# yuanming-hu/exposure

Measured on AMD Instinct MI355X. Metric: Mpixels/s through 8-step filter chain fwd+bwd, higher is better.
Workload: dtype f16; 1 GPU; 8-step filter chain (E,G,W,S+,T,Ct,BW,C) fwd+bwd, 64x512x512x3 f16 NHWC per GPU, one HIP kernel per filter step and direction; batch_per_gpu=64, global_batch=64, height=512, width=512, parallelism=image-sharded replicas x1 (no data-path collective), weak scaling, launch=hipGraph replay, 10 steps (330 captured launches) per replay, chain_streams=2, transport=none (one process)

## Files before the change

### exposure_amd/csrc/chain_steps.hip

```cpp
#include <hip/hip_runtime.h>
#include <stdint.h>

#include "../../include/exposure_hip.h"
#include "filter_math.h"
#include "pixel_io.h"
#include "kernel_common.h"
#include "host_common.h"

namespace expo {

struct ChainStepsFwdArgs {
  const void* x;
  void* y[kChainFuseMax];
  const float* prm[kChainFuseMax];
  int id[kChainFuseMax];
  int steps, hw;
};

template <typename T, class IO>
__global__ __launch_bounds__(kThreads) void chain_steps_fwd_kernel(const ChainStepsFwdArgs a) {
  constexpr int PPL = PixTraits<T>::PPL;
  const int n = blockIdx.y;
  const int hw = a.hw;
  const size_t off = size_t(n) * hw * 3;
  const int lane = threadIdx.x & 63;
  __shared__ float2_lut ftab[kWaves][32];
  float2_lut* const tab = ftab[threadIdx.x >> 6];
#if EXPO_FP16_OVFL
  if constexpr (sizeof(T) == 2) __builtin_amdgcn_s_setreg(1 | (23 << 6) | (0 << 11), 1);
#endif
  const __amdgpu_buffer_rsrc_t rx = make_image_rsrc(static_cast<const T*>(a.x) + off, hw);
  const int stride = gridDim.x * kThreads;
  for (int gw = blockIdx.x * kThreads + (threadIdx.x & ~63); gw * PPL < hw; gw += stride) {
    const int boff = chunk_byte_offset<T>(gw, lane);
    RawGroup cur = load_raw<IO::kLoadX>(rx, boff);
#pragma unroll 1
    for (int st = 0; st < a.steps; ++st) {
      const float* const prm = a.prm[st];
      float v[PPL * 3];
#define EXPO_CASE(ID, F)                               \
  case ID: {                                           \
    const typename F::Prm q = F::load(prm + n * F::NP); \
    unpack<T>(cur, v);                                 \
    _Pragma("unroll") for (int k = 0; k < PPL; ++k) {  \
      float y[3];                                      \
      F::fwd(q, v + 3 * k, y);                         \
      _Pragma("unroll") for (int c = 0; c < 3; ++c) v[3 * k + c] = y[c]; \
    }                                                  \
    cur = pack<T>(v);                                  \
  } break;
      switch (a.id[st]) {
        EXPO_CASE(0, ExposureF)
        EXPO_CASE(1, GammaF)
        EXPO_CASE(2, WhiteBalanceF)
        EXPO_CASE(3, SatPlusF)
        case 4:
          curve_lut_build<1>(prm[n * ToneF::NP + lane % ToneF::NP], tab);
          unpack<T>(cur, v);
          curve_lut_apply<1, PPL>(v, tab);
          cur = pack<T>(v);
          __builtin_amdgcn_wave_barrier();
          break;
        EXPO_CASE(5, ContrastF)
        EXPO_CASE(6, WnbF)
        case 7:
          curve_lut_build<3>(prm[n * ColorF::NP + lane % ColorF::NP], tab);
          unpack<T>(cur, v);
          curve_lut_apply<3, PPL>(v, tab);
          cur = pack<T>(v);
          __builtin_amdgcn_wave_barrier();
          break;
        EXPO_CASE(8, LevelF)
        default: break;
      }
#undef EXPO_CASE
      store_raw<IO::kStore>(make_image_rsrc(static_cast<T*>(a.y[st]) + off, hw), boff, cur);
    }
  }
}

template <typename T>
static int chain_steps_fwd_t(const ChainStepsFwdArgs& a, int np, int h, int w, int n_geom, hipStream_t s) {
  const Geom g = make_geom<T>(n_geom, h, w, {}, kGeomMap);
  const dim3 grid(g.blocks_x, np), block(kThreads);
  if (g.stream)
    hipLaunchKernelGGL((chain_steps_fwd_kernel<T, IoStream>), grid, block, 0, s, a);
  else
    hipLaunchKernelGGL((chain_steps_fwd_kernel<T, IoCached>), grid, block, 0, s, a);
  HIP_TRY(hipGetLastError(), "chain_steps_fwd launch");
  return EXPO_OK;
}

bool chain_steps_vec_path(void* const* acts, int steps, int h, int w, int dtype) {
  const int ppv = dtype == EXPO_F16 ? VecTraits<half_t>::PPV : VecTraits<float>::PPV;
  if ((long(h) * w) % ppv != 0) return false;
  for (int k = 0; k <= steps; ++k)
    if ((reinterpret_cast<uintptr_t>(acts[k]) & 3) != 0) return false;
  return true;
}

int chain_steps_fwd(const int* ids, int cnt, void* const* acts, const float* const* params, int nb, int np, int h,
                    int w, int dtype, int n_geom, hipStream_t s) {
  if (cnt < 1 || cnt > kChainFuseMax) return fail(EXPO_E_BADARG, "chain_steps_fwd: step count");
  const size_t ioff = size_t(nb) * h * w * 3 * (dtype == EXPO_F16 ? 2 : 4);
  ChainStepsFwdArgs a{};
  a.x = static_cast<const char*>(acts[0]) + ioff;
  for (int k = 0; k < cnt; ++k) {
    a.y[k] = static_cast<char*>(acts[k + 1]) + ioff;
    a.prm[k] = params[k] + size_t(nb) * kNumParams[ids[k]];
    a.id[k] = ids[k];
  }
  a.steps = cnt;
  a.hw = h * w;
  return dtype == EXPO_F16 ? chain_steps_fwd_t<half_t>(a, np, h, w, n_geom, s)
                           : chain_steps_fwd_t<float>(a, np, h, w, n_geom, s);
}

}
```

### exposure_amd/csrc/chain_steps_bwd.hip

```cpp
#include <hip/hip_runtime.h>
#include <stdint.h>

#include "../../include/exposure_hip.h"
#include "filter_math.h"
#include "pixel_io.h"
#include "kernel_common.h"
#include "host_common.h"
#include "stream_bodies.h"
#include "chain_steps_bwd_body.h"

namespace expo {

bool chain_steps_bwd_fusable(int id, int dtype, int mode) {
  if (id == 3 && dtype == EXPO_F32 && mode == 1) return false;
  return chain_steps_bwd_acc_floats(id) > 0;
}

int chain_steps_bwd_acc_floats(int id) {
  switch (id) {
#define EXPO_CASE(ID, F) \
  case ID: return kAccParts * F::NACC;
    EXPO_RUN_FILTERS(EXPO_CASE)
#undef EXPO_CASE
  }
  return 0;
}

template <typename T, int MODE, class IO, int NS>
__global__ __launch_bounds__(kThreads EXPO_BWD_MIN_WAVES) void chain_steps_bwd_kernel(const ChainStepsBwdArgs<NS> a) {
  constexpr int PPL = PixTraits<T>::PPL;
  static_assert(PPL >= kAccParts, "kParts == kAccParts in both storage types");
  const int n = blockIdx.y;
  const int hw = a.hw;
  const size_t off = size_t(n) * hw * 3;
  const int lane = threadIdx.x & 63;
#if EXPO_FP16_OVFL
  if constexpr (sizeof(T) == 2) __builtin_amdgcn_s_setreg(1 | (23 << 6) | (0 << 11), 1);
#endif
  const int stride = gridDim.x * kThreads;
  int gw = blockIdx.x * kThreads + (threadIdx.x & ~63);
  const bool work = gw * PPL < hw;
  const __amdgpu_buffer_rsrc_t rdy = make_image_rsrc(static_cast<const T*>(a.dy) + off, hw);
  int boff = chunk_byte_offset<T>(gw, lane);
  RawGroup cur, x[NS];
  if (work) {
    cur = load_raw<IO::kLoadDy>(rdy, boff);
#pragma unroll
    for (int k = 0; k < NS; ++k)
      x[k] = load_raw<IO::kLoadX>(make_image_rsrc(static_cast<const T*>(a.x[k]) + off, hw), boff);
  }
  extern __shared__ float accs[];
  float* const mine = accs + threadIdx.x;
  for (int f = 0; f < a.acc_floats; ++f) mine[f * kThreads] = 0.f;
  if (work) {
    while (true) {
      const int gn = gw + stride;
      const bool more = gn * PPL < hw;
      const int bnext = chunk_byte_offset<T>(gn, lane);
      RawGroup nxt = cur;
      if (more) nxt = load_raw<IO::kLoadDy>(rdy, bnext);
#pragma unroll 1
      for (int st = 0; st < NS; ++st) {
        const float* const prm = a.prm[st];
        float* const lds = mine + a.acc_at[st] * kThreads;
#define EXPO_CASE(ID, F) \
  case ID: run_step<F, T, MODE>(prm + n * F::NP, x[0], cur, lds); break;
        switch (a.id[st]) {
          EXPO_RUN_FILTERS(EXPO_CASE)
          default: break;
        }
#undef EXPO_CASE
        store_raw<IO::kStore>(make_image_rsrc(static_cast<T*>(a.dx[st]) + off, hw), boff, cur);
#pragma unroll
        for (int k = 0; k + 1 < NS; ++k) x[k] = x[k + 1];
        if (more) x[NS - 1] = load_raw<IO::kLoadX>(make_image_rsrc(static_cast<const T*>(a.x[st]) + off, hw), bnext);
      }
      if (!more) break;
      gw = gn;
      boff = bnext;
      cur = nxt;
    }
  }
#pragma unroll 1
  for (int st = 0; st < NS; ++st) {
    if (st > 0) __syncthreads();
    float* const rec = a.rec[st] + size_t(n) * gridDim.x * kWsSlots;
    const float* const lds = mine + a.acc_at[st] * kThreads;
#define EXPO_CASE(ID, F) \
  case ID: run_reduce<F, T>(lds, rec); break;
    switch (a.id[st]) {
      EXPO_RUN_FILTERS(EXPO_CASE)
      default: break;
    }
#undef EXPO_CASE
  }
}

template <typename T, int MODE, int NS>
static int chain_steps_bwd_launch(const ChainStepsBwdArgs<NS>& a, const Geom& g, int np, hipStream_t s) {
  const dim3 grid(g.blocks_x, np), block(kThreads);
  const size_t lds = size_t(a.acc_floats) * kThreads * sizeof(float);
  if (g.stream)
    hipLaunchKernelGGL((chain_steps_bwd_kernel<T, MODE, IoStream, NS>), grid, block, lds, s, a);
  else
    hipLaunchKernelGGL((chain_steps_bwd_kernel<T, MODE, IoCached, NS>), grid, block, lds, s, a);
  HIP_TRY(hipGetLastError(), "chain_steps_bwd launch");
  return EXPO_OK;
}

template <typename T, int NS>
static int chain_steps_bwd_t(const int* ids, int i0, void* const* acts, void* const* grads,
                             const float* const* params, float* records, size_t step_floats, int nb, int np, int h,
                             int w, int mode, int n_geom, hipStream_t s) {
  const Geom g = make_geom<T>(n_geom, h, w, {}, kGeomReduce);
  const size_t ioff = size_t(nb) * h * w * 3 * sizeof(T);
  ChainStepsBwdArgs<NS> a{};
  a.dy = static_cast<const char*>(grads[i0 + 1]) + ioff;
  for (int k = 0; k < NS; ++k) {
    const int i = i0 - k;
    a.x[k] = static_cast<const char*>(acts[i]) + ioff;
    a.dx[k] = static_cast<char*>(grads[i]) + ioff;
    a.prm[k] = params[i] + size_t(nb) * kNumParams[ids[i]];
    a.rec[k] = records + size_t(i) * step_floats + size_t(nb) * g.blocks_x * kWsSlots;
    a.id[k] = ids[i];
    a.acc_at[k] = a.acc_floats;
    a.acc_floats += chain_steps_bwd_acc_floats(ids[i]);
  }
  a.hw = h * w;
  return mode == 1 ? chain_steps_bwd_launch<T, 1, NS>(a, g, np, s) : chain_steps_bwd_launch<T, 0, NS>(a, g, np, s);
}

int chain_steps_bwd(const int* ids, int i0, int cnt, void* const* acts, void* const* grads,
                    const float* const* params, float* records, size_t step_floats, int nb, int np, int h, int w,
                    int dtype, int mode, int n_geom, hipStream_t s) {
  if (cnt < 2 || cnt > kChainFuseMax || cnt > i0 + 1) return fail(EXPO_E_BADARG, "chain_steps_bwd: step count");
  int acc_floats = 0;
  for (int k = 0; k < cnt; ++k) {
    if (!chain_steps_bwd_fusable(ids[i0 - k], dtype, mode) || !grads[i0 - k])
      return fail(EXPO_E_BADARG, "chain_steps_bwd: not a step of the run table with a dx");
    acc_floats += chain_steps_bwd_acc_floats(ids[i0 - k]);
  }
  if (acc_floats > kChainBwdAccFloatsMax) return fail(EXPO_E_BADARG, "chain_steps_bwd: accumulators of the run");
#define EXPO_GO(NS)                                                                                                   \
  case NS:                                                                                                            \
    return dtype == EXPO_F16                                                                                          \
               ? chain_steps_bwd_t<half_t, NS>(ids, i0, acts, grads, params, records, step_floats, nb, np, h, w, mode, \
                                               n_geom, s)                                                             \
               : chain_steps_bwd_t<float, NS>(ids, i0, acts, grads, params, records, step_floats, nb, np, h, w, mode,  \
                                              n_geom, s);
  switch (cnt) {
    EXPO_GO(2) EXPO_GO(3) EXPO_GO(4) EXPO_GO(5) EXPO_GO(6) EXPO_GO(7) EXPO_GO(8)
  }
#undef EXPO_GO
  static_assert(kChainFuseMax == 8, "one instantiation per run length");
  return fail(EXPO_E_BADARG, "chain_steps_bwd: step count");
}

}
```

### exposure_amd/csrc/chain_steps_bwd_body.h

```cpp
#pragma once
#include <hip/hip_runtime.h>
#include <stdint.h>

#include "filter_math.h"
#include "pixel_io.h"
#include "kernel_common.h"
#include "stream_bodies.h"

namespace expo {

template <int NS>
struct ChainStepsBwdArgs {
  const void* dy;
  const void* x[NS];
  void* dx[NS];
  const float* prm[NS];
  float* rec[NS];
  int id[NS];
  int acc_at[NS];
  int acc_floats, hw;
};

template <class F, typename T, int MODE>
__device__ __forceinline__ void run_step(const float* prm, const RawGroup& x, RawGroup& g, float* lds) {
  constexpr int PPL = PixTraits<T>::PPL;
  constexpr int kParts = kAccParts < PPL ? kAccParts : PPL;
  static_assert(!F::kHasGroupBwd && F::kLutFloats == 0, "element-wise filters only");
  const typename F::Prm q = F::load(prm);
  float a[kParts][F::NACC];
#pragma unroll
  for (int p = 0; p < kParts; ++p)
#pragma unroll
    for (int j = 0; j < F::NACC; ++j) a[p][j] = lds[(p * F::NACC + j) * kThreads];
  float v[PPL * 3], d[PPL * 3];
  unpack<T>(x, v);
  unpack<T>(g, d);
#pragma unroll
  for (int k = 0; k < PPL; ++k) {
    float dx[3];
    F::bwd(q, nullptr, v + 3 * k, d + 3 * k, dx, a[k % kParts], MODE);
#pragma unroll
    for (int c = 0; c < 3; ++c) d[3 * k + c] = dx[c];
  }
  g = pack<T>(d);
#pragma unroll
  for (int p = 0; p < kParts; ++p)
#pragma unroll
    for (int j = 0; j < F::NACC; ++j) lds[(p * F::NACC + j) * kThreads] = a[p][j];
}

template <class F, typename T>
__device__ __forceinline__ void run_reduce(const float* lds, float* rec) {
  constexpr int PPL = PixTraits<T>::PPL;
  constexpr int kParts = kAccParts < PPL ? kAccParts : PPL;
  float acc[F::NACC];
#pragma unroll
  for (int j = 0; j < F::NACC; ++j) acc[j] = lds[j * kThreads];
#pragma unroll
  for (int p = 0; p < kParts - 1; ++p)
#pragma unroll
    for (int j = 0; j < F::NACC; ++j) acc[j] += lds[((p + 1) * F::NACC + j) * kThreads];
  block_reduce_record<F::NACC>(acc, rec);
}

#define EXPO_RUN_FILTERS(X) X(0, ExposureF) X(1, GammaF) X(2, WhiteBalanceF) X(3, SatPlusF) X(8, LevelF)

}
```

### exposure_amd/csrc/chain_steps_bwd_rc.hip

```cpp
#include <hip/hip_runtime.h>
#include <stdint.h>

#include "../../include/exposure_hip.h"
#include "filter_math.h"
#include "pixel_io.h"
#include "kernel_common.h"
#include "host_common.h"
#include "stream_bodies.h"
#include "chain_steps_bwd_body.h"

namespace expo {

#define EXPO_RC_FILTERS(X) \
  X(0, ExposureF, 1, 1) X(1, GammaF, 1, 1) X(2, WhiteBalanceF, 1, 1) X(3, SatPlusF, 1, 1) X(8, LevelF, 1, 1)

template <typename T>
__host__ __device__ constexpr bool rc_recomputable(int id) {
  switch (id) {
#define EXPO_CASE(ID, F, H, S) \
  case ID: return sizeof(T) == 2 ? H : S;
    EXPO_RC_FILTERS(EXPO_CASE)
#undef EXPO_CASE
  }
  return false;
}

template <typename T>
__host__ __device__ constexpr bool rc_keeps_load(int id) {
  switch (id) {
#define EXPO_CASE(ID, F, H, S) \
  case ID: return !(sizeof(T) == 2 ? H : S);
    EXPO_RC_FILTERS(EXPO_CASE)
#undef EXPO_CASE
  }
  return false;
}

bool chain_steps_bwd_recomputes(int id, int dtype) {
  return dtype == EXPO_F16 ? rc_recomputable<half_t>(id) : rc_recomputable<float>(id);
}

template <typename T>
__device__ __forceinline__ RawGroup rc_forward(int id, const float* prm, int n, const RawGroup in, RawGroup out) {
  constexpr int PPL = PixTraits<T>::PPL;
#define EXPO_CASE(ID, F, H, S)                                           \
  case ID:                                                               \
    if constexpr (rc_recomputable<T>(ID)) {                              \
      const typename F::Prm q = F::load(prm + n * F::NP);                \
      float v[PPL * 3];                                                  \
      unpack<T>(in, v);                                                  \
      _Pragma("unroll") for (int k = 0; k < PPL; ++k) {                  \
        float y[3];                                                      \
        F::fwd(q, v + 3 * k, y);                                         \
        _Pragma("unroll") for (int c = 0; c < 3; ++c) v[3 * k + c] = y[c]; \
      }                                                                  \
      out = pack<T>(v);                                                  \
    }                                                                    \
    break;
  switch (id) {
    EXPO_RC_FILTERS(EXPO_CASE)
    default: break;
  }
#undef EXPO_CASE
  return out;
}

template <typename T, int NS, int K>
__device__ __forceinline__ void rc_sweep(const ChainStepsBwdArgs<NS>& a, int n, RawGroup (&x)[NS]) {
  if constexpr (K >= 0) {
    int s = K + 1;
    asm volatile("" : "+s"(s));
    x[K] = rc_forward<T>(a.id[s], a.prm[s], n, x[K + 1], x[K]);
    rc_sweep<T, NS, K - 1>(a, n, x);
  }
}

template <typename T, class IO, int NS>
__device__ __forceinline__ void rc_load_kept(const ChainStepsBwdArgs<NS>& a, size_t off, int hw, int boff,
                                             RawGroup (&x)[NS]) {
#pragma unroll
  for (int k = 0; k + 1 < NS; ++k)
    if (rc_keeps_load<T>(a.id[k + 1]))
      x[k] = load_raw<IO::kLoadX>(make_image_rsrc(static_cast<const T*>(a.x[k]) + off, hw), boff);
}

template <typename T, int MODE, class IO, int NS>
__global__ __launch_bounds__(kThreads EXPO_BWD_MIN_WAVES) void chain_steps_bwd_rc_kernel(const ChainStepsBwdArgs<NS> a) {
  constexpr int PPL = PixTraits<T>::PPL;
  static_assert(PPL >= kAccParts, "kParts == kAccParts in both storage types");
  const int n = blockIdx.y;
  const int hw = a.hw;
  const size_t off = size_t(n) * hw * 3;
  const int lane = threadIdx.x & 63;
#if EXPO_FP16_OVFL
  if constexpr (sizeof(T) == 2) __builtin_amdgcn_s_setreg(1 | (23 << 6) | (0 << 11), 1);
#endif
  const int stride = gridDim.x * kThreads;
  int gw = blockIdx.x * kThreads + (threadIdx.x & ~63);
  const bool work = gw * PPL < hw;
  const __amdgpu_buffer_rsrc_t rdy = make_image_rsrc(static_cast<const T*>(a.dy) + off, hw);
  const __amdgpu_buffer_rsrc_t rlow = make_image_rsrc(static_cast<const T*>(a.x[NS - 1]) + off, hw);
  int boff = chunk_byte_offset<T>(gw, lane);
  RawGroup cur, x[NS];
  if (work) {
    cur = load_raw<IO::kLoadDy>(rdy, boff);
    x[NS - 1] = load_raw<IO::kLoadX>(rlow, boff);
    rc_load_kept<T, IO, NS>(a, off, hw, boff, x);
  }
  extern __shared__ float accs[];
  float* const mine = accs + threadIdx.x;
  for (int f = 0; f < a.acc_floats; ++f) mine[f * kThreads] = 0.f;
  if (work) {
    while (true) {
      const int gn = gw + stride;
      const bool more = gn * PPL < hw;
      const int bnext = chunk_byte_offset<T>(gn, lane);
      RawGroup nxt = cur, nlow = x[NS - 1];
      if (more) {
        nxt = load_raw<IO::kLoadDy>(rdy, bnext);
        nlow = load_raw<IO::kLoadX>(rlow, bnext);
      }
      rc_sweep<T, NS, NS - 2>(a, n, x);
#pragma unroll 1
      for (int st = 0; st < NS; ++st) {
        const float* const prm = a.prm[st];
        float* const lds = mine + a.acc_at[st] * kThreads;
#define EXPO_CASE(ID, F) \
  case ID: run_step<F, T, MODE>(prm + n * F::NP, x[0], cur, lds); break;
        switch (a.id[st]) {
          EXPO_RUN_FILTERS(EXPO_CASE)
          default: break;
        }
#undef EXPO_CASE
        store_raw<IO::kStore>(make_image_rsrc(static_cast<T*>(a.dx[st]) + off, hw), boff, cur);
#pragma unroll
        for (int k = 0; k + 1 < NS; ++k) x[k] = x[k + 1];
      }
      if (!more) break;
      gw = gn;
      boff = bnext;
      cur = nxt;
      x[NS - 1] = nlow;
      rc_load_kept<T, IO, NS>(a, off, hw, boff, x);
    }
  }
#pragma unroll 1
  for (int st = 0; st < NS; ++st) {
    if (st > 0) __syncthreads();
    float* const rec = a.rec[st] + size_t(n) * gridDim.x * kWsSlots;
    const float* const lds = mine + a.acc_at[st] * kThreads;
#define EXPO_CASE(ID, F) \
  case ID: run_reduce<F, T>(lds, rec); break;
    switch (a.id[st]) {
      EXPO_RUN_FILTERS(EXPO_CASE)
      default: break;
    }
#undef EXPO_CASE
  }
}

template <typename T, int MODE, int NS>
static int chain_steps_bwd_rc_launch(const ChainStepsBwdArgs<NS>& a, const Geom& g, int np, hipStream_t s) {
  const dim3 grid(g.blocks_x, np), block(kThreads);
  const size_t lds = size_t(a.acc_floats) * kThreads * sizeof(float);
  if (g.stream)
    hipLaunchKernelGGL((chain_steps_bwd_rc_kernel<T, MODE, IoStream, NS>), grid, block, lds, s, a);
  else
    hipLaunchKernelGGL((chain_steps_bwd_rc_kernel<T, MODE, IoCached, NS>), grid, block, lds, s, a);
  HIP_TRY(hipGetLastError(), "chain_steps_bwd_rc launch");
  return EXPO_OK;
}

template <typename T, int NS>
static int chain_steps_bwd_rc_t(const int* ids, int i0, void* const* acts, void* const* grads,
                                const float* const* params, float* records, size_t step_floats, int nb, int np, int h,
                                int w, int mode, int n_geom, hipStream_t s) {
  const Geom g = make_geom<T>(n_geom, h, w, {}, kGeomReduce);
  const size_t ioff = size_t(nb) * h * w * 3 * sizeof(T);
  ChainStepsBwdArgs<NS> a{};
  a.dy = static_cast<const char*>(grads[i0 + 1]) + ioff;
  for (int k = 0; k < NS; ++k) {
    const int i = i0 - k;
    a.x[k] = static_cast<const char*>(acts[i]) + ioff;
    a.dx[k] = static_cast<char*>(grads[i]) + ioff;
    a.prm[k] = params[i] + size_t(nb) * kNumParams[ids[i]];
    a.rec[k] = records + size_t(i) * step_floats + size_t(nb) * g.blocks_x * kWsSlots;
    a.id[k] = ids[i];
    a.acc_at[k] = a.acc_floats;
    a.acc_floats += chain_steps_bwd_acc_floats(ids[i]);
  }
  a.hw = h * w;
  return mode == 1 ? chain_steps_bwd_rc_launch<T, 1, NS>(a, g, np, s) : chain_steps_bwd_rc_launch<T, 0, NS>(a, g, np, s);
}

int chain_steps_bwd_rc(const int* ids, int i0, int cnt, void* const* acts, void* const* grads,
                       const float* const* params, float* records, size_t step_floats, int nb, int np, int h, int w,
                       int dtype, int mode, int n_geom, hipStream_t s) {
  if (cnt < 2 || cnt > kChainFuseMax || cnt > i0 + 1) return fail(EXPO_E_BADARG, "chain_steps_bwd_rc: step count");
  int acc_floats = 0;
  for (int k = 0; k < cnt; ++k) {
    if (!chain_steps_bwd_fusable(ids[i0 - k], dtype, mode) || !grads[i0 - k])
      return fail(EXPO_E_BADARG, "chain_steps_bwd_rc: not a step of the run table with a dx");
    acc_floats += chain_steps_bwd_acc_floats(ids[i0 - k]);
  }
  if (acc_floats > kChainBwdAccFloatsMax) return fail(EXPO_E_BADARG, "chain_steps_bwd_rc: accumulators of the run");
#define EXPO_GO(NS)                                                                                                      \
  case NS:                                                                                                               \
    return dtype == EXPO_F16                                                                                             \
               ? chain_steps_bwd_rc_t<half_t, NS>(ids, i0, acts, grads, params, records, step_floats, nb, np, h, w, mode, \
                                                  n_geom, s)                                                             \
               : chain_steps_bwd_rc_t<float, NS>(ids, i0, acts, grads, params, records, step_floats, nb, np, h, w, mode,  \
                                                 n_geom, s);
  switch (cnt) {
    EXPO_GO(2) EXPO_GO(3) EXPO_GO(4) EXPO_GO(5) EXPO_GO(6) EXPO_GO(7) EXPO_GO(8)
  }
#undef EXPO_GO
  static_assert(kChainFuseMax == 8, "one instantiation per run length");
  return fail(EXPO_E_BADARG, "chain_steps_bwd_rc: step count");
}

}
```

Before: 37520 Mpixels/s.

## Scalarize parameter loads, prefetch LUT knots to LDS, pin occupancy and reorder stores

Filter parameters are read through the constant address space so the compiler can use scalar loads instead of per-lane vector loads. The forward kernel pre-stages the curve knot values for all steps into LDS once per block and pins waves-per-EU to 5. The backward kernel makes the loop-continue flag wave-uniform, adds empty asm barriers that pin loaded registers in place, and moves each gradient store after the next-x prefetch to overlap memory traffic. The extra LDS per wave, the forced occupancy, and the asm constraints may raise register pressure or cause spills.

Result: no change. 37650 Mpixels/s (median of 2 runs) (+0.3%).

```diff
diff --git a/exposure_amd/csrc/chain_steps.hip b/exposure_amd/csrc/chain_steps.hip
--- a/exposure_amd/csrc/chain_steps.hip
+++ b/exposure_amd/csrc/chain_steps.hip
@@ -17,8 +17,23 @@
   int steps, hw;
 };
 
+template <class F>
+__device__ __forceinline__ typename F::Prm load_prm_scalar(const float* p) {
+  const __attribute__((address_space(4))) float* const c = (const __attribute__((address_space(4))) float*)p;
+  float raw[F::NP];
+#pragma unroll
+  for (int j = 0; j < F::NP; ++j) raw[j] = c[j];
+  return F::load(raw);
+}
+
+__device__ __forceinline__ void settle(RawGroup& r) {
+#pragma unroll
+  for (int j = 0; j < 4; ++j) asm volatile("" : "+v"(r.q[j]));
+}
+
 template <typename T, class IO>
-__global__ __launch_bounds__(kThreads) void chain_steps_fwd_kernel(const ChainStepsFwdArgs a) {
+__global__ __launch_bounds__(kThreads) __attribute__((amdgpu_waves_per_eu(5, 5))) void chain_steps_fwd_kernel(
+    const ChainStepsFwdArgs a) {
   constexpr int PPL = PixTraits<T>::PPL;
   const int n = blockIdx.y;
   const int hw = a.hw;
@@ -26,6 +41,20 @@
   const int lane = threadIdx.x & 63;
   __shared__ float2_lut ftab[kWaves][32];
   float2_lut* const tab = ftab[threadIdx.x >> 6];
+  __shared__ float fknot[kWaves][kChainFuseMax][64];
+  float(*const knot)[64] = fknot[threadIdx.x >> 6];
+  {
+    float kv[kChainFuseMax];
+#pragma unroll
+    for (int st = 0; st < kChainFuseMax; ++st) {
+      const int id = a.id[st];
+      const int at = id == 4 ? n * ToneF::NP + lane % ToneF::NP : n * ColorF::NP + lane % ColorF::NP;
+      const float* const p = st < a.steps ? a.prm[st] : a.prm[0];
+      kv[st] = p[id == 4 || id == 7 ? at : 0];
+    }
+#pragma unroll
+    for (int st = 0; st < kChainFuseMax; ++st) knot[st][lane] = kv[st];
+  }
 #if EXPO_FP16_OVFL
   if constexpr (sizeof(T) == 2) __builtin_amdgcn_s_setreg(1 | (23 << 6) | (0 << 11), 1);
 #endif
@@ -34,13 +63,14 @@
   for (int gw = blockIdx.x * kThreads + (threadIdx.x & ~63); gw * PPL < hw; gw += stride) {
     const int boff = chunk_byte_offset<T>(gw, lane);
     RawGroup cur = load_raw<IO::kLoadX>(rx, boff);
+    settle(cur);
 #pragma unroll 1
     for (int st = 0; st < a.steps; ++st) {
       const float* const prm = a.prm[st];
       float v[PPL * 3];
 #define EXPO_CASE(ID, F)                               \
   case ID: {                                           \
-    const typename F::Prm q = F::load(prm + n * F::NP); \
+    const typename F::Prm q = load_prm_scalar<F>(prm + n * F::NP); \
     unpack<T>(cur, v);                                 \
     _Pragma("unroll") for (int k = 0; k < PPL; ++k) {  \
       float y[3];                                      \
@@ -55,7 +85,7 @@
         EXPO_CASE(2, WhiteBalanceF)
         EXPO_CASE(3, SatPlusF)
         case 4:
-          curve_lut_build<1>(prm[n * ToneF::NP + lane % ToneF::NP], tab);
+          curve_lut_build<1>(knot[st][lane], tab);
           unpack<T>(cur, v);
           curve_lut_apply<1, PPL>(v, tab);
           cur = pack<T>(v);
@@ -64,7 +94,7 @@
         EXPO_CASE(5, ContrastF)
         EXPO_CASE(6, WnbF)
         case 7:
-          curve_lut_build<3>(prm[n * ColorF::NP + lane % ColorF::NP], tab);
+          curve_lut_build<3>(knot[st][lane], tab);
           unpack<T>(cur, v);
           curve_lut_apply<3, PPL>(v, tab);
           cur = pack<T>(v);
diff --git a/exposure_amd/csrc/chain_steps_bwd.hip b/exposure_amd/csrc/chain_steps_bwd.hip
--- a/exposure_amd/csrc/chain_steps_bwd.hip
+++ b/exposure_amd/csrc/chain_steps_bwd.hip
@@ -55,10 +55,13 @@
   if (work) {
     while (true) {
       const int gn = gw + stride;
-      const bool more = gn * PPL < hw;
+      const bool more = __builtin_amdgcn_readfirstlane(gn * PPL < hw);
       const int bnext = chunk_byte_offset<T>(gn, lane);
       RawGroup nxt = cur;
       if (more) nxt = load_raw<IO::kLoadDy>(rdy, bnext);
+      settle(cur);
+#pragma unroll
+      for (int k = 0; k < NS; ++k) settle(x[k]);
 #pragma unroll 1
       for (int st = 0; st < NS; ++st) {
         const float* const prm = a.prm[st];
@@ -70,10 +73,10 @@
           default: break;
         }
 #undef EXPO_CASE
-        store_raw<IO::kStore>(make_image_rsrc(static_cast<T*>(a.dx[st]) + off, hw), boff, cur);
 #pragma unroll
         for (int k = 0; k + 1 < NS; ++k) x[k] = x[k + 1];
         if (more) x[NS - 1] = load_raw<IO::kLoadX>(make_image_rsrc(static_cast<const T*>(a.x[st]) + off, hw), bnext);
+        store_raw<IO::kStore>(make_image_rsrc(static_cast<T*>(a.dx[st]) + off, hw), boff, cur);
       }
       if (!more) break;
       gw = gn;
diff --git a/exposure_amd/csrc/chain_steps_bwd_body.h b/exposure_amd/csrc/chain_steps_bwd_body.h
--- a/exposure_amd/csrc/chain_steps_bwd_body.h
+++ b/exposure_amd/csrc/chain_steps_bwd_body.h
@@ -21,12 +21,26 @@
   int acc_floats, hw;
 };
 
+template <class F>
+__device__ __forceinline__ typename F::Prm load_prm_scalar(const float* p) {
+  const __attribute__((address_space(4))) float* const c = (const __attribute__((address_space(4))) float*)p;
+  float raw[F::NP];
+#pragma unroll
+  for (int j = 0; j < F::NP; ++j) raw[j] = c[j];
+  return F::load(raw);
+}
+
+__device__ __forceinline__ void settle(RawGroup& r) {
+#pragma unroll
+  for (int j = 0; j < 4; ++j) asm volatile("" : "+v"(r.q[j]));
+}
+
 template <class F, typename T, int MODE>
 __device__ __forceinline__ void run_step(const float* prm, const RawGroup& x, RawGroup& g, float* lds) {
   constexpr int PPL = PixTraits<T>::PPL;
   constexpr int kParts = kAccParts < PPL ? kAccParts : PPL;
   static_assert(!F::kHasGroupBwd && F::kLutFloats == 0, "element-wise filters only");
-  const typename F::Prm q = F::load(prm);
+  const typename F::Prm q = load_prm_scalar<F>(prm);
   float a[kParts][F::NACC];
 #pragma unroll
   for (int p = 0; p < kParts; ++p)
diff --git a/exposure_amd/csrc/chain_steps_bwd_rc.hip b/exposure_amd/csrc/chain_steps_bwd_rc.hip
--- a/exposure_amd/csrc/chain_steps_bwd_rc.hip
+++ b/exposure_amd/csrc/chain_steps_bwd_rc.hip
@@ -46,7 +46,7 @@
 #define EXPO_CASE(ID, F, H, S)                                           \
   case ID:                                                               \
     if constexpr (rc_recomputable<T>(ID)) {                              \
-      const typename F::Prm q = F::load(prm + n * F::NP);                \
+      const typename F::Prm q = load_prm_scalar<F>(prm + n * F::NP);     \
       float v[PPL * 3];                                                  \
       unpack<T>(in, v);                                                  \
       _Pragma("unroll") for (int k = 0; k < PPL; ++k) {                  \
```
